# techshoww/RoMa

Measured on AMD Instinct MI355X. Metric: image-pairs/sec at 560->864, higher is better.
Workload: dtype fp16; 1 GPU; roma_outdoor 560->864 full coarse-to-fine symmetric match (BASELINE configs[1]; configs[2] = --pairs 8 --gpus 8); launch=eager launches, coarse_res=560, upsample_res=864, parallelism=single GPU

## Files before the change

include/roma_hip.h:

```cpp
#ifndef ROMA_HIP_H
#define ROMA_HIP_H

#include <stdint.h>

#ifdef __cplusplus
extern "C" {
#endif

#define ROMA_ABI_VERSION 5

enum { ROMA_F32 = 0, ROMA_F16 = 1, ROMA_BF16 = 2 };
enum { ROMA_NCHW = 0, ROMA_NHWC = 1 };
enum { ROMA_LC_AUTO = 0, ROMA_LC_TILE8X4 = 1, ROMA_LC_TILE8X8 = 2, ROMA_LC_ROWS8 = 3 };
enum { ROMA_E_ARG = -1, ROMA_E_DTYPE = -2, ROMA_E_SHAPE = -3, ROMA_E_ALIGN = -4, ROMA_E_UNSUPPORTED = -5 };

int roma_abi_version(void);
const char* roma_last_error(void);

int roma_local_corr(const void* f0, const void* f1, const float* flow, void* out,
                    int B, int C, int H, int W, int r, int dtype,
                    int layout, int f0_pitch, int f1_pitch, int out_layout, int out_pitch, int f1_batch_shift, int variant,
                    void* stream);

int roma_warp_bilinear(const void* src, const float* flow, void* dst,
                       int B, int C, int Hs, int Ws, int H, int W, int dtype,
                       int layout, int src_pitch, int dst_layout, int dst_pitch, int src_batch_shift, void* stream);

int roma_disp_emb(const float* flow, const float* weight, const float* bias, void* dst,
                  int B, int E, int H, int W, float gain, int dtype, int dst_layout, int dst_pitch, void* stream);

int roma_interp_bilinear(const float* x, float* y, int N, int Hi, int Wi, int Ho, int Wo, void* stream);

int roma_flow_update(float* flow, float* cert, const float* cert_in, const float* delta,
                     int B, int H, int W, float sx, float sy, void* stream);

int roma_cls_to_flow_refine(const void* logits, float* flow_out, float* cert_out,
                            int B, int C, int HW, long stride_b, long stride_c, long stride_p,
                            int dtype, void* stream);

int roma_cos_kernel(const void* x, const void* y, float* K, int B, int N, int M, int D, int dtype, int x_pitch, int y_pitch,
                    int y_batch_shift, float T, float eps, float diag_add, void* stream);

int roma_chol_diag_block(float* A, int lda, long strideA, float* W, int ldw, long strideW, int nb, int B, int* info,
                         int info_base, void* stream);

int roma_chol_step(float* A, int lda, long strideA, int n, int ncols, int j, int nb, const float* W, int ldw, long strideW, float* R,
                   int ldr, long strideR, float* Wn, int ldwn, long strideWn, int* info, int info_base, int B, void* stream);

int roma_chol_subst_step(int dir, const float* W, int ldw, long strideW, const float* R, long strideRb, long strideRs, int ldr, float* T,
                         long strideTb, long strideTs, int ldt, int t_in_panel, float* X, int ldx, long strideX, int n, int m, int nb,
                         int s, int B, void* stream);

int roma_attention_fwd(const void* q, const void* k, const void* v, void* o, int B, int H, int Nq, int Nk, int head_dim, long q_sb,
                       long q_sn, long q_sh, long k_sb, long k_sn, long k_sh, long v_sb, long v_sn, long v_sh, long o_sb, long o_sn,
                       long o_sh, float scale, int dtype, void* stream);

int roma_match_finalize(const float* flow, const float* cert, const float* cert16, float* warp, float* certainty,
                        int P, int H, int W, int H16, int W16, int symmetric, void* stream);

int roma_kde_density(const float* x, float* density, int N, int down, float std, int half_mode, void* stream);

int roma_race_keys(const float* p, const long* counter, float* keys, long N, float thresh, unsigned seed, unsigned stage,
                   void* stream);

int roma_nn_argmin(const float* q, const float* r, int* idx, int NQ, int NR, void* stream);

int roma_resample_u8(const void* in, void* out, int H, int W, int C, int out_size, int axis, const int* bounds,
                     const int* coef, int ksize, void* stream);
int roma_normalize_u8(const void* in, float* out, int H, int W, const float* mean3, const float* std3, void* stream);

int roma_bias_relu_nchw(void* x, const void* bias, int B, int C, int HW, int dtype, void* stream);

int roma_bias_relu_pool2_nchw(void* x, const void* bias, void* pooled, int B, int C, int H, int W, int dtype, void* stream);

int roma_bias_relu_nhwc(void* x, const void* bias, long npix, int C, int dtype, void* stream);
int roma_bias_relu_pool2_nhwc(void* x, const void* bias, void* pooled, int B, int C, int H, int W, int dtype, void* stream);

int roma_dwconv5x5_bn_relu(const void* x, const float* w, const float* scale, const float* shift, void* y,
                           int B, int C, int H, int W, int dtype, int x_pitch, int y_pitch, void* stream);

int roma_refiner_block(const void* x, const void* w25, const float* scale, const float* shift, const void* wt,
                       const float* bias, void* y, int B, int C, int H, int W, int kpad, int dtype, int x_pitch, int y_pitch,
                       void* stream);

int roma_refiner_wide_pack(const void* wt, void* wp, int D);
int roma_refiner_wide_taps(const void* w25, void* w25p, int D);
int roma_refiner_block_wide(const void* x, const void* w25p, const float* scale, const float* shift, const void* wp,
                            const float* bias, void* y, int B, int H, int W, int D, int x_pitch, int y_pitch, int dtype,
                            void* stream);

int roma_pointwise_mfma(const void* x, const void* wt, const float* bias, void* y, long M, int C, int kpad, int dtype,
                        int x_pitch, int y_pitch, void* stream);

int roma_refiner_head(const void* x, const float* wo, const float* bo, float* flow, const float* cert_in, float* cert_out,
                      float* delta_out, int B, int H, int W, int C, int pitch, int dtype, float sx, float sy, void* stream);

int roma_pointwise_small(const void* x, const float* wt, const float* bias, void* y, long M, int C, int dtype,
                         int x_pitch, int y_pitch, void* stream);

int roma_add_layernorm(void* x, int x_dtype, long x_stride, const void* y, int y_dtype, long y_stride, const float* ls,
                       const float* gamma, const float* beta, void* out, int out_dtype, long out_stride, long rows, int C,
                       float eps, void* stream);

int roma_tiny_corr_posembed(const float* f0, const float* f1, float* out, int B, int C,
                            int H0, int W0, int H1, int W1, int exact, void* stream);

int roma_jpeg_info(const void* data, long nbytes, int* info);
int roma_jpeg_entropy_decode(const void* data, long nbytes, int16_t* coef, uint16_t* qt);
int roma_jpeg_reconstruct(const int16_t* coef, const uint16_t* qt, void* planes, void* rgb, const int* info, void* stream);

long roma_ransac_workspace(int kind, int P, int N, int iters, long* offsets);
int roma_ransac_hypotheses(int kind, const double* xa, const double* xb, int P, int N, int iters, float threshold, unsigned seed,
                           int p0, void* ws, long ws_bytes, void* stream);
int roma_ransac_select(int kind, const double* xa, const double* xb, int P, int N, int iters, float threshold, int lo_iters,
                       const void* ws, long ws_bytes, double* model, unsigned char* mask, void* stream);

#ifdef __cplusplus
}
#endif
#endif
```

roma_amd/_lib.py:

```python
from __future__ import annotations

import ctypes
import os
from ctypes import c_char_p, c_float, c_int, c_long, c_void_p

_HERE = os.path.dirname(os.path.abspath(__file__))
LIB_PATH = os.path.join(_HERE, "csrc", "libroma_hip.so")

ROMA_F32, ROMA_F16, ROMA_BF16 = 0, 1, 2
ROMA_NCHW, ROMA_NHWC = 0, 1
LC_VARIANTS = {"auto": 0, "tile8x4": 1, "tile8x8": 2, "rows8": 3}
ABI_VERSION = 5
ROMA_E_ARG, ROMA_E_DTYPE, ROMA_E_SHAPE, ROMA_E_ALIGN, ROMA_E_UNSUPPORTED = -1, -2, -3, -4, -5

SIGNATURES = {
    "roma_abi_version": [],
    "roma_last_error": [],
    "roma_local_corr": [c_void_p, c_void_p, c_void_p, c_void_p, c_int, c_int, c_int, c_int, c_int, c_int,
                        c_int, c_int, c_int, c_int, c_int, c_int, c_int, c_void_p],
    "roma_warp_bilinear": [c_void_p, c_void_p, c_void_p, c_int, c_int, c_int, c_int, c_int, c_int, c_int,
                           c_int, c_int, c_int, c_int, c_int, c_void_p],
    "roma_disp_emb": [c_void_p, c_void_p, c_void_p, c_void_p, c_int, c_int, c_int, c_int, c_float, c_int, c_int, c_int, c_void_p],
    "roma_interp_bilinear": [c_void_p, c_void_p, c_int, c_int, c_int, c_int, c_int, c_void_p],
    "roma_flow_update": [c_void_p, c_void_p, c_void_p, c_void_p, c_int, c_int, c_int, c_float, c_float, c_void_p],
    "roma_cls_to_flow_refine": [c_void_p, c_void_p, c_void_p, c_int, c_int, c_int, c_long, c_long, c_long, c_int, c_void_p],
    "roma_cos_kernel": [c_void_p, c_void_p, c_void_p, c_int, c_int, c_int, c_int, c_int, c_int, c_int, c_int, c_float, c_float,
                        c_float, c_void_p],
    "roma_add_layernorm": [c_void_p, c_int, c_long, c_void_p, c_int, c_long, c_void_p, c_void_p, c_void_p, c_void_p, c_int, c_long,
                           c_long, c_int, c_float, c_void_p],
    "roma_attention_fwd": [c_void_p, c_void_p, c_void_p, c_void_p, c_int, c_int, c_int, c_int, c_int] + [c_long] * 12 + [c_float, c_int, c_void_p],
    "roma_chol_diag_block": [c_void_p, c_int, c_long, c_void_p, c_int, c_long, c_int, c_int, c_void_p, c_int, c_void_p],
    "roma_chol_step": [c_void_p, c_int, c_long, c_int, c_int, c_int, c_int, c_void_p, c_int, c_long, c_void_p, c_int, c_long,
                       c_void_p, c_int, c_long, c_void_p, c_int, c_int, c_void_p],
    "roma_chol_subst_step": [c_int, c_void_p, c_int, c_long, c_void_p, c_long, c_long, c_int, c_void_p, c_long, c_long, c_int, c_int,
                             c_void_p, c_int, c_long, c_int, c_int, c_int, c_int, c_int, c_void_p],
    "roma_match_finalize": [c_void_p, c_void_p, c_void_p, c_void_p, c_void_p, c_int, c_int, c_int, c_int, c_int, c_int, c_void_p],
    "roma_kde_density": [c_void_p, c_void_p, c_int, c_int, c_float, c_int, c_void_p],
    "roma_nn_argmin": [c_void_p, c_void_p, c_void_p, c_int, c_int, c_void_p],
    "roma_race_keys": [c_void_p, c_void_p, c_void_p, c_long, c_float, ctypes.c_uint, ctypes.c_uint, c_void_p],
    "roma_dwconv5x5_bn_relu": [c_void_p, c_void_p, c_void_p, c_void_p, c_void_p, c_int, c_int, c_int, c_int, c_int, c_int, c_int, c_void_p],
    "roma_resample_u8": [c_void_p, c_void_p, c_int, c_int, c_int, c_int, c_int, c_void_p, c_void_p, c_int, c_void_p],
    "roma_normalize_u8": [c_void_p, c_void_p, c_int, c_int, c_void_p, c_void_p, c_void_p],
    "roma_bias_relu_nchw": [c_void_p, c_void_p, c_int, c_int, c_int, c_int, c_void_p],
    "roma_bias_relu_pool2_nchw": [c_void_p, c_void_p, c_void_p, c_int, c_int, c_int, c_int, c_int, c_void_p],
    "roma_bias_relu_nhwc": [c_void_p, c_void_p, c_long, c_int, c_int, c_void_p],
    "roma_bias_relu_pool2_nhwc": [c_void_p, c_void_p, c_void_p, c_int, c_int, c_int, c_int, c_int, c_void_p],
    "roma_pointwise_mfma": [c_void_p, c_void_p, c_void_p, c_void_p, c_long, c_int, c_int, c_int, c_int, c_int, c_void_p],
    "roma_refiner_block": [c_void_p, c_void_p, c_void_p, c_void_p, c_void_p, c_void_p, c_void_p, c_int, c_int, c_int, c_int, c_int, c_int,
                           c_int, c_int, c_void_p],
    "roma_refiner_wide_pack": [c_void_p, c_void_p, c_int],
    "roma_refiner_wide_taps": [c_void_p, c_void_p, c_int],
    "roma_jpeg_info": [c_void_p, c_long, c_void_p],
    "roma_jpeg_entropy_decode": [c_void_p, c_long, c_void_p, c_void_p],
    "roma_jpeg_reconstruct": [c_void_p, c_void_p, c_void_p, c_void_p, c_void_p, c_void_p],
    "roma_refiner_block_wide": [c_void_p, c_void_p, c_void_p, c_void_p, c_void_p, c_void_p, c_void_p, c_int, c_int, c_int, c_int, c_int, c_int,
                                c_int, c_void_p],
    "roma_refiner_head": [c_void_p, c_void_p, c_void_p, c_void_p, c_void_p, c_void_p, c_void_p, c_int, c_int, c_int, c_int, c_int, c_int,
                          c_float, c_float, c_void_p],
    "roma_pointwise_small": [c_void_p, c_void_p, c_void_p, c_void_p, c_long, c_int, c_int, c_int, c_int, c_void_p],
    "roma_tiny_corr_posembed": [c_void_p, c_void_p, c_void_p, c_int, c_int, c_int, c_int, c_int, c_int, c_int, c_void_p],
    "roma_ransac_workspace": [c_int, c_int, c_int, c_int, c_void_p],
    "roma_ransac_hypotheses": [c_int, c_void_p, c_void_p, c_int, c_int, c_int, c_float, ctypes.c_uint, c_int, c_void_p, c_long, c_void_p],
    "roma_ransac_select": [c_int, c_void_p, c_void_p, c_int, c_int, c_int, c_float, c_int, c_void_p, c_long, c_void_p, c_void_p,
                           c_void_p],
}
_RESTYPES = {"roma_last_error": c_char_p, "roma_ransac_workspace": c_long}

_lib = None


class RomaHipError(RuntimeError):
    pass


def load() -> ctypes.CDLL:
    global _lib
    if _lib is not None:
        return _lib
    if not os.path.exists(LIB_PATH):
        raise RomaHipError(f"{LIB_PATH} is missing: build it with `python -c 'import __graft_entry__ as g; g.build()'` "
                           f"or `make -C roma_amd/csrc`.  roma_amd has no CPU/PyTorch fallback for its kernels.")
    lib = ctypes.CDLL(LIB_PATH)
    for name, argtypes in SIGNATURES.items():
        fn = getattr(lib, name)
        fn.argtypes = argtypes
        fn.restype = _RESTYPES.get(name, c_int)
    if lib.roma_abi_version() != ABI_VERSION:
        raise RomaHipError(f"libroma_hip.so ABI {lib.roma_abi_version()} != binding ABI {ABI_VERSION}")
    _lib = lib
    return lib


def check(rc: int, what: str):
    if rc == 0:
        return
    msg = load().roma_last_error().decode(errors="replace")
    if rc < 0:
        raise ValueError(f"{what}: {msg} (code {rc})")
    raise RomaHipError(f"{what}: HIP error {rc}: {msg}")
```

roma_amd/matcher.py:

```python
from __future__ import annotations

import math
import os
from typing import Dict, Optional
from warnings import warn

import numpy as np
import torch
import torch.nn as nn
import torch.nn.functional as F

from . import ops
from .transformer import Block, TransformerDecoder

IMAGENET_MEAN = (0.485, 0.456, 0.406)
IMAGENET_STD = (0.229, 0.224, 0.225)


def _round_up(n, m):
    return (n + m - 1) // m * m


def pixel_grid(b, h, w, device):
    ys = torch.linspace(-1 + 1 / h, 1 - 1 / h, h, device=device)
    xs = torch.linspace(-1 + 1 / w, 1 - 1 / w, w, device=device)
    return torch.stack((xs[None, :].expand(h, w), ys[:, None].expand(h, w)), dim=0)[None].expand(b, 2, h, w).contiguous()


def _params_version(module):
    return tuple((p.data_ptr(), 0 if p.is_inference() else p._version) for p in list(module.parameters()) + list(module.buffers()))


def _zero_pad(t, *shape):
    out = torch.zeros(shape, dtype=t.dtype, device=t.device)
    out[tuple(slice(0, s) for s in t.shape)] = t
    return out


class ConvRefiner(nn.Module):

    def __init__(self, in_dim, hidden_dim, out_dim, hidden_blocks, displacement_emb_dim, local_corr_radius=None,
                 amp_dtype=torch.float16):
        super().__init__()
        assert in_dim == hidden_dim, "depthwise refiner blocks keep the channel count (all shipped models)"

        def block(i, o):
            return nn.Sequential(nn.Conv2d(i, o, 5, 1, 2, groups=i), nn.BatchNorm2d(o), nn.ReLU(inplace=True), nn.Conv2d(o, o, 1, 1, 0))

        self.block1 = block(in_dim, hidden_dim)
        self.hidden_blocks = nn.Sequential(*[block(hidden_dim, hidden_dim) for _ in range(hidden_blocks)])
        self.out_conv = nn.Conv2d(hidden_dim, out_dim, 1, 1, 0)
        self.disp_emb = nn.Conv2d(2, displacement_emb_dim, 1, 1, 0)
        self.has_displacement_emb = True
        self.local_corr_radius = local_corr_radius
        self.in_dim, self.out_dim = in_dim, out_dim
        self.amp_dtype = amp_dtype
        self._prep = None

    def prepare(self, dtype):
        key = (dtype, _params_version(self))
        if self._prep is not None and self._prep[0] == key:
            return self._prep[1]
        D = self.in_dim
        Dp = _round_up(D, 64) if D > 160 else _round_up(D, 8)
        dev = self.out_conv.weight.device
        fuse_max = int(os.environ.get("ROMA_FUSED_BLOCK", "32"))
        fused = Dp <= min(fuse_max, 160) and dtype in (torch.float16, torch.bfloat16)
        mid = (not fused) and 32 < Dp <= 160 and dtype in (torch.float16, torch.bfloat16) and os.environ.get("ROMA_PW_MFMA", "1") != "0"
        wide = Dp == 576 and dtype == torch.float16 and os.environ.get("ROMA_WIDE_BLOCK", "1") != "0"
        blocks = []
        for blk in [self.block1] + list(self.hidden_blocks):
            dw, bn, _, pw = blk
            s = bn.weight.float() / torch.sqrt(bn.running_var.float() + bn.eps)
            w25 = torch.zeros(25, Dp, device=dev)
            w25[:, :D] = dw.weight.float().reshape(D, 25).t()
            scale = torch.zeros(Dp, device=dev)
            shift = torch.zeros(Dp, device=dev)
            scale[:D] = s
            b_dw = dw.bias.float() if dw.bias is not None else torch.zeros(D, device=dev)
            shift[:D] = (b_dw - bn.running_mean.float()) * s + bn.bias.float()
            wt = torch.zeros(Dp, Dp, device=dev)
            wt[:D, :D] = pw.weight.float().reshape(D, D).t()
            b = torch.zeros(Dp, device=dev)
            b[:D] = pw.bias.float()
            if wide:
                blocks.append((w25.contiguous(), scale, shift, wt.to(dtype).contiguous(), b.to(dtype),
                               ops.refiner_wide_taps(w25, dtype), ops.refiner_wide_pack(wt.t().contiguous().to(dtype)), b.contiguous()))
            elif fused:
                kp = 32 if Dp <= 32 else 160
                blocks.append((_zero_pad(w25, 25, kp).to(dtype), _zero_pad(scale, kp), _zero_pad(shift, kp),
                               _zero_pad(wt.t(), kp, kp).to(dtype), _zero_pad(b, kp)))
            elif mid:
                blocks.append((w25.contiguous(), scale, shift, _zero_pad(wt.t(), 160, 160).to(dtype), _zero_pad(b, 160)))
            elif Dp <= 32:
                blocks.append((w25.contiguous(), scale, shift, wt.contiguous(), b.contiguous()))
            else:
                blocks.append((w25.contiguous(), scale, shift, wt.to(dtype).contiguous(), b.to(dtype)))
        wo = torch.zeros(Dp, self.out_dim, device=dev)
        wo[:D] = self.out_conv.weight.float().reshape(self.out_dim, D).t()
        prep = dict(D=D, Dp=Dp, fused=fused, mid=mid, wide=wide, blocks=blocks, wo=wo.contiguous(), bo=self.out_conv.bias.float(),
                    we=self.disp_emb.weight.float().reshape(-1, 2).contiguous(), be=self.disp_emb.bias.float())
        self._prep = (key, prep)
        return prep

    def new_buffer(self, B, h, w, dtype, device):
        return torch.empty((B, h, w, self.prepare(dtype)["Dp"]), dtype=dtype, device=device)

    @torch.no_grad()
    def _body(self, x, y, flow, scale_factor, dtype, buf=None, batch_shift=0):
        P = self.prepare(dtype)
        B, C, h, w = x.shape
        D, Dp = P["D"], P["Dp"]
        E = P["we"].shape[0]
        r = self.local_corr_radius
        K = (2 * r + 1) ** 2 if r else 0
        assert 2 * C + E + K == D, "feature width does not match this refiner"
        x_in_place = buf is not None
        if buf is None:
            buf = torch.empty((B, h, w, Dp), dtype=dtype, device=x.device)
        assert buf.shape == (B, h, w, Dp) and buf.dtype == dtype and buf.is_contiguous()
        d = buf.permute(0, 3, 1, 2)
        if x_in_place:
            assert x.data_ptr() == buf.data_ptr() and x.stride(1) == 1, "x must already be channels [0, C) of buf"
        else:
            d[:, :C].copy_(x)
        if Dp > D:
            buf[..., D:].zero_()
        yy = y.to(dtype)
        ops.warp_bilinear(yy, flow, out=d[:, C:2 * C], batch_shift=batch_shift)
        ops.disp_emb(flow, P["we"], P["be"], 40 / 32 * scale_factor, out=d[:, 2 * C:2 * C + E])
        if r:
            ops.local_correlation(d[:, :C], yy, r, flow=flow, out=d[:, 2 * C + E:D], batch_shift=batch_shift)
        M = B * h * w
        cur = buf
        if P["wide"] and B * ((h + 7) // 8) * ((w + 15) // 16) >= 2 * 256:
            nxt = torch.empty_like(buf)
            for blk in P["blocks"]:
                ops.refiner_block_wide(cur, blk[5], blk[1], blk[2], blk[6], blk[7], out=nxt)
                cur, nxt = nxt, cur
            return cur, P
        if P["fused"]:
            nxt = torch.empty_like(buf)
            for (w25, scale, shift, wt, b) in P["blocks"]:
                ops.refiner_block(cur, w25, scale, shift, wt, b, Dp, out=nxt)
                cur, nxt = nxt, cur
            return cur, P
        for blk in P["blocks"]:
            w25, scale, shift, wt, b = blk[:5]
            t = ops.dwconv5x5_bn_relu(cur.permute(0, 3, 1, 2), w25, scale, shift)
            rows = t.permute(0, 2, 3, 1).reshape(M, Dp)
            if P["mid"]:
                cur = ops.pointwise_mfma(rows, wt, b, Dp)
            else:
                cur = ops.pointwise_small(rows, wt, b) if Dp <= 32 else torch.addmm(b, rows, wt)
            cur = cur.view(B, h, w, Dp)
        return cur, P

    @torch.no_grad()
    def forward(self, x, y, flow, scale_factor=1, logits=None, dtype=None):
        flow = flow.float().contiguous()
        cur, P = self._body(x, y, flow, scale_factor, dtype or self.amp_dtype)
        B, h, w, Dp = cur.shape
        out = torch.addmm(P["bo"], cur.reshape(B * h * w, Dp).float(), P["wo"])
        out = out.view(B, h, w, self.out_dim).permute(0, 3, 1, 2).contiguous()
        return out[:, :-1], out[:, -1:]

    @torch.no_grad()
    def forward_update(self, x, y, flow, certainty, scale_factor, sx, sy, dtype=None, buf=None, batch_shift=0):
        cur, P = self._body(x, y, flow, scale_factor, dtype or self.amp_dtype, buf=buf, batch_shift=batch_shift)
        return ops.refiner_head(cur, P["wo"], P["bo"], flow, certainty, sx, sy)


class CosKernel(nn.Module):
    def __init__(self, T=0.2, learn_temperature=False):
        super().__init__()
        self.T = T

    def __call__(self, x, y, eps=1e-6):
        return ops.cos_kernel(x, y, T=self.T, eps=eps)


class GP(nn.Module):

    def __init__(self, gp_dim=512, T=0.2, sigma_noise=0.1, kernel=None, **_):
        super().__init__()
        self.K = CosKernel(T=T)
        self.sigma_noise = sigma_noise
        self.pos_conv = nn.Conv2d(2, gp_dim, 1, 1)
        self.dim = gp_dim
        self._basis = {}

    def basis(self, b, h, w, device):
        key = (h, w, device, _params_version(self.pos_conv))
        f = self._basis.get(key)
        if f is None:
            g = pixel_grid(1, h, w, device)
            f = torch.cos(8 * math.pi * F.conv2d(g, self.pos_conv.weight.float(), self.pos_conv.bias.float()))
            f = f.flatten(2).transpose(1, 2).contiguous()
            self._basis = {key: f}
        return f.expand(b, -1, -1)

    @torch.no_grad()
    def forward(self, x, y, **kwargs):
        b, c, h1, w1 = x.shape
        _, _, h2, w2 = y.shape
        xs = x.float().flatten(2).transpose(1, 2).contiguous()
        ys = y.float().flatten(2).transpose(1, 2).contiguous()
        K_yy = ops.cos_kernel(ys, ys, T=self.K.T, diag_add=self.sigma_noise)
        K_xy = ops.cos_kernel(xs, ys, T=self.K.T)
        mu = self.posterior_product(K_xy, ops.spd_solve(K_yy, self.basis(1, h2, w2, x.device)))
        return mu.transpose(1, 2).reshape(b, self.dim, h1, w1)

    def posterior_rows(self, xs, ys, h2, w2, fp64=False, batch_shift=0, out=None, check="now"):
        B, n = xs.shape[0], xs.shape[1]
        s = batch_shift % B
        basis = self.basis(1, h2, w2, xs.device)
        if fp64:
            a = xs.double()
            c = (a.roll(-s, 0) if s else a) if ys is None else ys.double()

            def cosk(u, v):
                g = torch.einsum("bnd,bmd->bnm", u, v) / (u.norm(dim=-1)[..., None] * v.norm(dim=-1)[:, None] + 1e-6)
                return ((g - 1.0) / self.K.T).exp()

            Kyy = cosk(c, c) + self.sigma_noise * torch.eye(c.shape[1], device=c.device, dtype=torch.float64)
            Z = torch.cholesky_solve(basis.double().expand(B, -1, -1), torch.linalg.cholesky(Kyy))
            mu = (cosk(a, c) @ Z).float()
            if out is not None:
                out.copy_(mu)
                return out
            return mu
        if ys is None:
            K_self = ops.cos_kernel(xs, xs, T=self.K.T, diag_add=self.sigma_noise)
            K_xy = ops.cos_kernel(xs, xs, T=self.K.T, batch_shift=s)
            Z = ops.spd_solve(K_self, basis, check=check)
            if s:
                assert 2 * s == B, "only the half swap of forward_symmetric"
                Z = torch.cat((Z[s:], Z[:s]), dim=0)
        else:
            K_yy = ops.cos_kernel(ys, ys, T=self.K.T, diag_add=self.sigma_noise)
            K_xy = ops.cos_kernel(xs, ys, T=self.K.T)
            Z = ops.spd_solve(K_yy, basis, check=check)
        return self.posterior_product(K_xy, Z, out)

    @staticmethod
    def posterior_product(K_xy, Z, out=None):
        mu = torch.bmm(K_xy.double(), Z.double())
        if out is None:
            return mu.float()
        out.copy_(mu)
        return out


class Decoder(nn.Module):
    def __init__(self, embedding_decoder, gps, proj, conv_refiner, detach=True, scales=("16", "8", "4", "2", "1"),
                 amp_dtype=torch.float16, **_):
        super().__init__()
        self.embedding_decoder, self.gps, self.proj, self.conv_refiner = embedding_decoder, gps, proj, conv_refiner
        self.scales = list(scales)
        self.refine_init = 4
        self.amp_dtype = amp_dtype
        self.gp_precision = "fp32"
        self.record = None
        self.flow_override = None
        self._proj = None

    def _embedding_decoder_for(self, dtype):
        if dtype == torch.float32:
            return self.embedding_decoder
        key = (dtype, _params_version(self.embedding_decoder))
        hit = self.__dict__.get("_embed_cast")
        if hit is None or hit[0] != key:
            import copy
            with torch.inference_mode(False), torch.no_grad():
                cp = copy.deepcopy(self.embedding_decoder).eval()
                for m in cp.modules():
                    if isinstance(m, nn.Linear):
                        m.to(dtype)
                hit = (key, cp)
            self.__dict__["_embed_cast"] = hit
        return hit[1]

    def get_placeholder_flow(self, b, h, w, device):
        return pixel_grid(b, h, w, device)

    def folded_proj(self, dtype):
        key = (dtype, _params_version(self.proj))
        if self._proj is not None and self._proj[0] == key:
            return self._proj[1]
        out = {}
        for s, seq in self.proj.items():
            conv, bn = seq[0], seq[1]
            g = bn.weight.float() / torch.sqrt(bn.running_var.float() + bn.eps)
            wt = (conv.weight.float().reshape(conv.out_channels, -1) * g[:, None]).t().contiguous().to(dtype)
            b = ((conv.bias.float() - bn.running_mean.float()) * g + bn.bias.float()).to(dtype)
            out[s] = (wt, b)
            if wt.shape[1] < 16:
# ... 348 lines not shown
```

roma_amd/ops.py:

```python
from __future__ import annotations

import math
from typing import Optional

import torch

from . import _lib
from ._lib import ROMA_BF16, ROMA_F16, ROMA_F32, ROMA_NCHW, ROMA_NHWC, check

_DT = {torch.float32: ROMA_F32, torch.float16: ROMA_F16, torch.bfloat16: ROMA_BF16}


class KernelTimer:

    def __init__(self):
        self.enabled = False
        self.bracket_overhead_s = 0.0
        self.records = []

    def start(self):
        self.records.clear()
        torch.cuda.synchronize()
        pairs = []
        for _ in range(32):
# ... 366 lines not shown
    p = p.reshape(-1).float().contiguous()
    if counter is not None:
        counter = counter.reshape(-1).long().contiguous()
        assert counter.numel() == p.numel()
    keys = torch.empty_like(p)
    check(_lib.load().roma_race_keys(_p(p), _p(counter), _p(keys), p.numel(), float(thresh), int(seed) & 0xFFFFFFFF,
                                     int(stage) & 0xFFFFFFFF, _stream()), "roma_race_keys")
    return keys


def nn_argmin(q, r):
    _need_gpu(q, r)
    if q.dim() != 2 or q.shape[1] != 2 or r.dim() != 2 or r.shape[1] != 2:
        raise ValueError("nn_argmin expects (N,2) point sets")
    q, r = q.float().contiguous(), r.float().contiguous()
    idx = torch.empty((q.shape[0],), dtype=torch.int32, device=q.device)
    check(_lib.load().roma_nn_argmin(_p(q), _p(r), _p(idx), q.shape[0], r.shape[0], _stream()), "roma_nn_argmin")
    return idx.long()


def dwconv5x5_bn_relu(x, w25, scale, shift, out=None):
    _need_gpu(x, w25, scale, shift, out)
    B, C, H, W = x.shape
    lx, px, xx = feat_layout(x)
    if lx != ROMA_NHWC:
        raise ValueError("dwconv5x5_bn_relu needs channels-last input")
    if out is None:
        out = nhwc_empty(B, C, H, W, x.dtype, x.device, pitch=px)
    lo, po, o = feat_layout(out)
    if lo != ROMA_NHWC or o is not out:
        raise ValueError("dwconv5x5_bn_relu needs channels-last output")
    check(_lib.load().roma_dwconv5x5_bn_relu(_p(xx), _p(w25), _p(scale), _p(shift), _p(out), B, C, H, W, _dt(xx), px, po, _stream()),
          "roma_dwconv5x5_bn_relu")
    return out


def resample_u8(img, out_size, axis, bounds, coef, ksize):
    _need_gpu(img, bounds, coef)
    H, W, C = img.shape
    assert img.dtype == torch.uint8 and img.is_contiguous() and bounds.dtype == torch.int32 and coef.dtype == torch.int32
    assert bounds.shape == (out_size, 2) and coef.shape == (out_size, ksize) and bounds.is_contiguous() and coef.is_contiguous()
    out = torch.empty((H, out_size, C) if axis else (out_size, W, C), dtype=torch.uint8, device=img.device)
    check(_lib.load().roma_resample_u8(_p(img), _p(out), H, W, C, out_size, axis, _p(bounds), _p(coef), ksize, _stream()), "roma_resample_u8")
    return out


def normalize_u8(img, mean, std):
    import ctypes
    _need_gpu(img)
    H, W, C = img.shape
    assert C == 3 and img.dtype == torch.uint8 and img.is_contiguous()
    out = torch.empty((3, H, W), dtype=torch.float32, device=img.device)
    m = (ctypes.c_float * 3)(*mean)
    s = (ctypes.c_float * 3)(*std)
    check(_lib.load().roma_normalize_u8(_p(img), _p(out), H, W, ctypes.cast(m, ctypes.c_void_p), ctypes.cast(s, ctypes.c_void_p), _stream()),
          "roma_normalize_u8")
    return out


def _is_nhwc(x):
    return x.dim() == 4 and x.shape[1] > 1 and x.stride(1) == 1 and x.is_contiguous(memory_format=torch.channels_last)


def bias_relu_(x, bias):
    _need_gpu(x, bias)
    B, C, H, W = x.shape
    assert bias.dtype == x.dtype and bias.numel() == C and bias.is_contiguous()
    if _is_nhwc(x):
        check(_lib.load().roma_bias_relu_nhwc(_p(x), _p(bias), B * H * W, C, _dt(x), _stream()), "roma_bias_relu_nhwc")
        return x
    assert x.is_contiguous()
    step = max(1, 65535 // C)
    for b0 in range(0, B, step):
        xb = x[b0:b0 + step]
        check(_lib.load().roma_bias_relu_nchw(_p(xb), _p(bias), xb.shape[0], C, H * W, _dt(x), _stream()), "roma_bias_relu_nchw")
    return x


def bias_relu_pool2_(x, bias):
    _need_gpu(x, bias)
    B, C, H, W = x.shape
    assert bias.dtype == x.dtype and bias.numel() == C and bias.is_contiguous() and H % 2 == 0 and W % 2 == 0
    if _is_nhwc(x):
        out = torch.empty((B, H // 2, W // 2, C), dtype=x.dtype, device=x.device).permute(0, 3, 1, 2)
        check(_lib.load().roma_bias_relu_pool2_nhwc(_p(x), _p(bias), _p(out), B, C, H, W, _dt(x), _stream()), "roma_bias_relu_pool2_nhwc")
        return out
    assert x.is_contiguous()
    out = torch.empty((B, C, H // 2, W // 2), dtype=x.dtype, device=x.device)
    step = max(1, 65535 // C)
    for b0 in range(0, B, step):
        xb = x[b0:b0 + step]
        check(_lib.load().roma_bias_relu_pool2_nchw(_p(xb), _p(bias), _p(out[b0:b0 + step]), xb.shape[0], C, H, W, _dt(x), _stream()),
              "roma_bias_relu_pool2_nchw")
    return out


def pointwise_mfma(rows, wt, bias, C, out=None):
    _need_gpu(rows, wt, bias, out)
    M, pitch = rows.shape
    kpad = wt.shape[0]
    assert rows.is_contiguous() and wt.is_contiguous() and wt.dtype == rows.dtype and bias.numel() == kpad and bias.dtype == torch.float32
    if out is None:
        out = torch.empty_like(rows)
    assert out.shape == rows.shape and out.is_contiguous()
    check(_lib.load().roma_pointwise_mfma(_p(rows), _p(wt), _p(bias), _p(out), M, C, kpad, _dt(rows), pitch, pitch, _stream()),
          "roma_pointwise_mfma")
    return out


def refiner_wide_pack(wt_out_in):
    w = wt_out_in.detach().to("cpu").contiguous()
    assert w.dim() == 2 and w.shape[0] == w.shape[1] and w.element_size() == 2
    out = torch.empty_like(w)
    check(_lib.load().roma_refiner_wide_pack(w.data_ptr(), out.data_ptr(), w.shape[0]), "roma_refiner_wide_pack")
    return out.to(wt_out_in.device)


def refiner_wide_taps(w25, dtype=torch.float16):
    D = w25.shape[1]
    w = w25.detach().to("cpu").to(dtype).contiguous()
    assert w.shape == (25, D) and w.element_size() == 2
    out = torch.empty((D // 32, 5, 4, 2, 6, 4, 2), dtype=dtype)
    check(_lib.load().roma_refiner_wide_taps(w.data_ptr(), out.data_ptr(), D), "roma_refiner_wide_taps")
    return out.to(w25.device)


def refiner_block_wide(x_nhwc, w25p, scale, shift, wp, bias, out=None):
    _need_gpu(x_nhwc, w25p, scale, shift, wp, bias, out)
    B, H, W, D = x_nhwc.shape
    assert x_nhwc.is_contiguous() and w25p.shape == (D // 32, 5, 4, 2, 6, 4, 2) and w25p.dtype == x_nhwc.dtype and w25p.is_contiguous()
    assert all(t.dtype == torch.float32 and t.numel() == D and t.is_contiguous() for t in (scale, shift, bias))
    if out is None:
        out = torch.empty_like(x_nhwc)
    assert out.shape == x_nhwc.shape and out.is_contiguous() and out.data_ptr() != x_nhwc.data_ptr()
    check(_lib.load().roma_refiner_block_wide(_p(x_nhwc), _p(w25p), _p(scale), _p(shift), _p(wp), _p(bias), _p(out), B, H, W, D, D, D,
                                              _dt(x_nhwc), _stream()), "roma_refiner_block_wide")
    return out


def refiner_block(x_nhwc, w25, scale, shift, wt, bias, C, out=None):
    _need_gpu(x_nhwc, w25, scale, shift, wt, bias, out)
    B, h, w, pitch = x_nhwc.shape
    kpad = wt.shape[0]
    assert x_nhwc.is_contiguous() and wt.is_contiguous() and w25.is_contiguous() and wt.dtype == x_nhwc.dtype == w25.dtype
    assert w25.shape == (25, kpad) and wt.shape == (kpad, kpad) and scale.numel() == shift.numel() == bias.numel() == kpad
    if out is None:
        out = torch.empty_like(x_nhwc)
    assert out.is_contiguous() and out.shape == x_nhwc.shape and out.data_ptr() != x_nhwc.data_ptr()
    check(_lib.load().roma_refiner_block(_p(x_nhwc), _p(w25), _p(scale), _p(shift), _p(wt), _p(bias), _p(out), B, C, h, w, kpad,
                                         _dt(x_nhwc), pitch, pitch, _stream()), "roma_refiner_block")
    return out


def refiner_head(x_nhwc, wo, bo, flow, certainty, sx, sy, want_delta=False):
    _need_gpu(x_nhwc, wo, bo, flow, certainty)
    B, h, w, pitch = x_nhwc.shape
    C = wo.shape[0]
    assert x_nhwc.is_contiguous() and flow.is_contiguous() and flow.dtype == torch.float32 and wo.is_contiguous()
    cert_in = None if certainty is None else certainty.float().contiguous()
    cert = torch.empty((B, 1, h, w), dtype=torch.float32, device=flow.device)
    delta = torch.empty((B, 3, h, w), dtype=torch.float32, device=flow.device) if want_delta else None
    check(_lib.load().roma_refiner_head(_p(x_nhwc), _p(wo), _p(bo), _p(flow), _p(cert_in), _p(cert), _p(delta), B, h, w, C, pitch,
                                        _dt(x_nhwc), float(sx), float(sy), _stream()), "roma_refiner_head")
    return (flow, cert, delta) if want_delta else (flow, cert)


def pointwise_small(x_rows, wt, bias, out=None):
    _need_gpu(x_rows, wt, bias, out)
    M, C = x_rows.shape
    assert x_rows.stride(1) == 1
    if out is None:
        out = torch.empty((M, C), dtype=x_rows.dtype, device=x_rows.device)
    check(_lib.load().roma_pointwise_small(_p(x_rows), _p(wt), _p(bias), _p(out), M, C, _dt(x_rows), x_rows.stride(0), out.stride(0),
                                           _stream()), "roma_pointwise_small")
    return out


def attention(qkv, n_valid=None, out=None):
    _need_gpu(qkv, out)
    B, N, three, H, d = qkv.shape
    assert three == 3 and qkv.is_contiguous()
    if out is None:
        out = torch.empty((B, N, H * d), dtype=qkv.dtype, device=qkv.device)
    assert out.is_contiguous() and out.shape == (B, N, H * d) and out.dtype == qkv.dtype
    es = qkv.element_size()
    sb, sn, sh = qkv.stride(0), qkv.stride(1), qkv.stride(3)
    base = qkv.data_ptr()
    step = qkv.stride(2) * es
    check(_lib.load().roma_attention_fwd(base, base + step, base + 2 * step, out.data_ptr(), B, H, N, N if n_valid is None else int(n_valid), d,
                                         sb, sn, sh, sb, sn, sh, sb, sn, sh, out.stride(0), out.stride(1), d, float(d) ** -0.5, _dt(qkv),
                                         _stream()), "roma_attention_fwd")
    return out


def add_layernorm(x, y, ln_weight, ln_bias, eps, out_dtype, ls=None):
    _need_gpu(x, y, ln_weight, ln_bias, ls)
    C = x.shape[-1]
    assert x.is_contiguous() and (y is None or (y.is_contiguous() and y.shape == x.shape))
    rows = x.numel() // C
    out = torch.empty(x.shape, dtype=out_dtype, device=x.device)
    for t in (ln_weight, ln_bias, ls):
        assert t is None or (t.dtype == torch.float32 and t.is_contiguous() and t.numel() == C)
    check(_lib.load().roma_add_layernorm(_p(x), _dt(x), C, _p(y), _dt(y) if y is not None else 0, C, _p(ls), _p(ln_weight), _p(ln_bias),
                                         _p(out), _DT[out_dtype], C, rows, C, float(eps), _stream()), "roma_add_layernorm")
    return out


def tiny_corr_posembed(f0, f1, exact=False):
    _need_gpu(f0, f1)
    B, C, H0, W0 = f0.shape
    _, _, H1, W1 = f1.shape
    a = f0.float().permute(0, 2, 3, 1).contiguous()
    b = f1.float().permute(0, 2, 3, 1).contiguous()
    out = torch.empty((B, 2, H0, W0), dtype=torch.float32, device=f0.device)
    TIMER.wrap("tiny_corr", 2.0 * B * H0 * W0 * H1 * W1 * C, f"C{C}_{H0}x{W0}",
               lambda: check(_lib.load().roma_tiny_corr_posembed(_p(a), _p(b), _p(out), B, C, H0, W0, H1, W1, 1 if exact else 0, _stream()),
                             "roma_tiny_corr_posembed"))
    return out
```

Before: 56.88 image-pairs/s.

## Fuse depthwise 5x5 conv, BN-ReLU and MFMA pointwise for mid-width refiner blocks

```diff
diff --git a/include/roma_hip.h b/include/roma_hip.h
--- a/include/roma_hip.h
+++ b/include/roma_hip.h
@@ -83,6 +83,9 @@
                        const float* bias, void* y, int B, int C, int H, int W, int kpad, int dtype, int x_pitch, int y_pitch,
                        void* stream);
 
+int roma_refiner_mid(const void* x, const float* w25, const float* scale, const float* shift, const void* wt,
+                     const float* bias, void* y, int B, int C, int H, int W, int dtype, int x_pitch, int y_pitch, void* stream);
+
 int roma_refiner_wide_pack(const void* wt, void* wp, int D);
 int roma_refiner_wide_taps(const void* w25, void* w25p, int D);
 int roma_refiner_block_wide(const void* x, const void* w25p, const float* scale, const float* shift, const void* wp,
diff --git a/roma_amd/_lib.py b/roma_amd/_lib.py
--- a/roma_amd/_lib.py
+++ b/roma_amd/_lib.py
@@ -48,6 +48,8 @@
     "roma_pointwise_mfma": [c_void_p, c_void_p, c_void_p, c_void_p, c_long, c_int, c_int, c_int, c_int, c_int, c_void_p],
     "roma_refiner_block": [c_void_p, c_void_p, c_void_p, c_void_p, c_void_p, c_void_p, c_void_p, c_int, c_int, c_int, c_int, c_int, c_int,
                            c_int, c_int, c_void_p],
+    "roma_refiner_mid": [c_void_p, c_void_p, c_void_p, c_void_p, c_void_p, c_void_p, c_void_p, c_int, c_int, c_int, c_int, c_int, c_int, c_int,
+                         c_void_p],
     "roma_refiner_wide_pack": [c_void_p, c_void_p, c_int],
     "roma_refiner_wide_taps": [c_void_p, c_void_p, c_int],
     "roma_jpeg_info": [c_void_p, c_long, c_void_p],
diff --git a/roma_amd/csrc/refiner_mid.hip b/roma_amd/csrc/refiner_mid.hip
--- /dev/null
+++ b/roma_amd/csrc/refiner_mid.hip
@@ -0,0 +1,288 @@
+#include <algorithm>
+#include <cstdlib>
+#include "common.h"
+
+namespace roma {
+namespace {
+
+typedef _Float16 h8v __attribute__((ext_vector_type(8)));
+
+constexpr int RM_NT = 512;
+constexpr int RM_KPAD = 160, RM_KS = 5;
+constexpr int RM_RS = RM_KPAD / 8 + 1;
+constexpr int RM_OS = RM_KPAD + 8;
+constexpr int RM_XT = 16;
+constexpr int RM_RMAX = 16;
+
+struct RMParams {
+  const half_t* x;
+  half_t* y;
+  const float* w25;
+  const half_t* wt;
+  const float* scale;
+  const float* shift;
+  const float* bias;
+  int B, H, W, C, x_pitch, y_pitch;
+  int R;
+  int tiles_x, tiles_y, ntile;
+};
+
+inline int rm_rows(int C, int xs, int ys) { return std::min(RM_RMAX, RM_NT / (C / 8) / (RM_XT / xs) * ys); }
+inline int rm_trows(int R) { return (R + 1) & ~1; }
+inline size_t rm_smem(int C, int R) {
+  return (size_t)RM_KPAD * RM_RS * 16 + (size_t)rm_trows(R) * RM_XT * RM_OS * 2 + (size_t)25 * C * 4 + (size_t)3 * RM_KPAD * 4;
+}
+
+template <int RM_XS, int RM_YS, int RM_PD>
+__global__ __launch_bounds__(RM_NT, 1) void refiner_mid_kernel(RMParams p) {
+  constexpr int RM_NC = RM_XS + 4, NSX = RM_XT / RM_XS;
+  extern __shared__ __attribute__((aligned(16))) unsigned char smem[];
+  u32x4* s_pw = reinterpret_cast<u32x4*>(smem);
+  half_t* s_t = reinterpret_cast<half_t*>(s_pw + RM_KPAD * RM_RS);
+  float* s_w = reinterpret_cast<float*>(s_t + ((p.R + 1) & ~1) * RM_XT * RM_OS);
+  float* s_cs = s_w + 25 * p.C;
+  const int tid = threadIdx.x, lane = tid & 63;
+  const int wv = __builtin_amdgcn_readfirstlane(tid >> 6);
+  const int m = lane & 15, kq = lane >> 4;
+  const int C = p.C, H = p.H, W = p.W, R = p.R;
+  const int PK = C >> 3;
+
+  for (int i = tid; i < RM_KPAD * (RM_KPAD / 8); i += RM_NT) {
+    const int n = i / (RM_KPAD / 8), k = i - n * (RM_KPAD / 8);
+    s_pw[n * RM_RS + k] = reinterpret_cast<const u32x4*>(p.wt)[i];
+  }
+  for (int i = tid; i < 25 * C / 4; i += RM_NT) reinterpret_cast<float4_t*>(s_w)[i] = reinterpret_cast<const float4_t*>(p.w25)[i];
+  for (int i = tid; i < RM_KPAD; i += RM_NT) {
+    s_cs[i] = i < C ? p.scale[i] : 0.f;
+    s_cs[RM_KPAD + i] = i < C ? p.shift[i] : 0.f;
+    s_cs[2 * RM_KPAD + i] = p.bias[i];
+  }
+  {
+    const int npad = RM_KPAD / 8 - PK;
+    for (int i = tid; i < R * RM_XT * npad; i += RM_NT) {
+      const int px = i / npad, k = PK + (i - px * npad);
+      *reinterpret_cast<u32x4*>(s_t + px * RM_OS + k * 8) = u32x4{0, 0, 0, 0};
+    }
+  }
+
+  int row, sx, k;
+  {
+    const int s = tid / PK;
+    k = tid - s * PK;
+    sx = s % NSX;
+    row = s / NSX * RM_YS;
+  }
+  const bool act = row < R;
+  if (!act) { row = 0; sx = 0; k = 0; }
+  const int c0 = k * 8;
+  const int tpix = row * RM_XT + sx * RM_XS;
+
+  const int ntile = p.ntile, tiles_per_img = p.tiles_x * p.tiles_y;
+  const bool xcd_order = (gridDim.x & 7) == 0 && ntile >= 64;
+  const int nx = xcd_order ? (int)(gridDim.x >> 3) : (int)gridDim.x;
+  const int band = xcd_order ? (ntile + 7) >> 3 : ntile;
+  const int t_beg = xcd_order ? (int)(blockIdx.x & 7) * band + (int)(blockIdx.x >> 3) : (int)blockIdx.x;
+  const int t_end = xcd_order ? min(((int)(blockIdx.x & 7) + 1) * band, ntile) : ntile;
+  auto tile_origin = [&](int tile, int& b, int& ty0, int& tx0) {
+    b = tile / tiles_per_img;
+    const int tt = tile - b * tiles_per_img, tyi = tt / p.tiles_x;
+    ty0 = tyi * R;
+    tx0 = (tt - tyi * p.tiles_x) * RM_XT;
+  };
+  const char* xc = reinterpret_cast<const char*>(p.x);
+  auto load_row_clamped = [&](u32x4 (&dst)[RM_NC], int b, int yi, int xi0) {
+    const unsigned ro = (unsigned)((b * H + min(max(yi, 0), H - 1)) * W);
+#pragma unroll
+    for (int cx = 0; cx < RM_NC; ++cx)
+      dst[cx] = *reinterpret_cast<const u32x4*>(xc + ((ro + (unsigned)min(max(xi0 + cx, 0), W - 1)) * (unsigned)p.x_pitch + (unsigned)c0) * 2u);
+  };
+
+  constexpr int NR = RM_YS + 4, PD = RM_PD;
+  u32x4 q[PD][RM_NC];
+  {
+    int b, ty0, tx0;
+    tile_origin(min(t_beg, ntile - 1), b, ty0, tx0);
+#pragma unroll
+    for (int j = 0; j < PD; ++j) load_row_clamped(q[j], b, ty0 + row + j - 2, tx0 + sx * RM_XS - 2);
+  }
+  __syncthreads();
+
+  const u32x4* t_rd = reinterpret_cast<const u32x4*>(s_t + (2 * wv * RM_XT + m) * RM_OS) + kq;
+  const u32x4* pw_rd = s_pw + m * RM_RS + kq;
+  const float* bias_rd = s_cs + 2 * RM_KPAD + m;
+  half_t* o_wr = s_t + (2 * wv * RM_XT + 4 * kq) * RM_OS + m;
+  const int NTL = (C + 15) >> 4;
+
+  for (int tile = t_beg; tile < t_end; tile += nx) {
+    int b, ty0, tx0;
+    tile_origin(tile, b, ty0, tx0);
+    const int ys = ty0 + row, xs = tx0 + sx * RM_XS;
+    float acc[RM_YS][RM_XS][8];
+#pragma unroll
+    for (int oy = 0; oy < RM_YS; ++oy)
+#pragma unroll
+      for (int o = 0; o < RM_XS; ++o)
+#pragma unroll
+        for (int e = 0; e < 8; ++e) acc[oy][o][e] = 0.f;
+    auto fma_row = [&](const u32x4 (&src)[RM_NC], int dy, float (&ac)[RM_XS][8]) {
+#pragma unroll
+      for (int hf = 0; hf < 2; ++hf) {
+        const float* wr = s_w + dy * 5 * C + c0 + 4 * hf;
+        float4_t w5[5];
+#pragma unroll
+        for (int dx = 0; dx < 5; ++dx) w5[dx] = *reinterpret_cast<const float4_t*>(wr + dx * C);
+#pragma unroll
+        for (int cx = 0; cx < RM_NC; ++cx) {
+          float f[4];
+#pragma unroll
+          for (int i = 0; i < 2; ++i) {
+            const uint32_t u = src[cx][2 * hf + i];
+            const half2_t h = __builtin_bit_cast(half2_t, u);
+            f[2 * i] = (float)h[0];
+            f[2 * i + 1] = (float)h[1];
+          }
+#pragma unroll
+          for (int dx = 0; dx < 5; ++dx) {
+            const int o = cx - dx;
+            if (o >= 0 && o < RM_XS) {
+#pragma unroll
+              for (int e = 0; e < 4; ++e) ac[o][4 * hf + e] = __builtin_fmaf(w5[dx][e], f[e], ac[o][4 * hf + e]);
+            }
+          }
+        }
+      }
+    };
+    auto mask_row = [&](u32x4 (&v)[RM_NC], int iy) {
+      const int yi = ys + iy - 2;
+      const bool oky = yi >= 0 && yi < H;
+#pragma unroll
+      for (int cx = 0; cx < RM_NC; ++cx) {
+        const int xi = xs - 2 + cx;
+        if (!(oky && xi >= 0 && xi < W)) v[cx] = u32x4{0, 0, 0, 0};
+      }
+    };
+    const bool interior = ty0 >= 2 && ty0 + R + 2 <= H && tx0 >= 2 && tx0 + RM_XT + 2 <= W;
+    int b2, ty2, tx2;
+    tile_origin(min(tile + nx, t_end - 1), b2, ty2, tx2);
+#pragma unroll 1
+    for (int iy = 0; iy < NR; ++iy) {
+      u32x4 cur[RM_NC];
+#pragma unroll
+      for (int cx = 0; cx < RM_NC; ++cx) cur[cx] = q[0][cx];
+#pragma unroll
+      for (int j = 0; j + 1 < PD; ++j)
+#pragma unroll
+        for (int cx = 0; cx < RM_NC; ++cx) q[j][cx] = q[j + 1][cx];
+      if (!interior) mask_row(cur, iy);
+      const bool mine = iy + PD < NR;
+      load_row_clamped(q[PD - 1], mine ? b : b2, (mine ? ty0 + iy + PD : ty2 + iy + PD - NR) + row - 2, (mine ? tx0 : tx2) + sx * RM_XS - 2);
+      __builtin_amdgcn_sched_barrier(0);
+#pragma unroll
+      for (int oy = 0; oy < RM_YS; ++oy) {
+        const int dy = iy - oy;
+        if (dy >= 0 && dy <= 4) fma_row(cur, dy, acc[oy]);
+      }
+    }
+    if (act) {
+      float sc[8], sh[8];
+#pragma unroll
+      for (int e = 0; e < 8; e += 4) {
+        *reinterpret_cast<float4_t*>(&sc[e]) = *reinterpret_cast<const float4_t*>(s_cs + c0 + e);
+        *reinterpret_cast<float4_t*>(&sh[e]) = *reinterpret_cast<const float4_t*>(s_cs + RM_KPAD + c0 + e);
+      }
+#pragma unroll
+      for (int oy = 0; oy < RM_YS; ++oy)
+#pragma unroll
+        for (int o = 0; o < RM_XS; ++o) {
+          float v[8];
+#pragma unroll
+          for (int e = 0; e < 8; ++e) v[e] = fmaxf(__builtin_fmaf(acc[oy][o][e], sc[e], sh[e]), 0.f);
+          *reinterpret_cast<u32x4*>(s_t + (tpix + oy * RM_XT + o) * RM_OS + c0) = pack16<half_t>(v);
+        }
+    }
+    __syncthreads();
+
+    if (2 * wv < R) {
+      u32x4 a[2][RM_KS];
+#pragma unroll
+      for (int i = 0; i < 2; ++i)
+#pragma unroll
+        for (int ks = 0; ks < RM_KS; ++ks) a[i][ks] = t_rd[i * (RM_XT * RM_OS / 8) + 4 * ks];
+      float4_t pr[2][RM_KPAD / 16];
+#pragma unroll
+      for (int nt = 0; nt < RM_KPAD / 16; ++nt) {
+        pr[0][nt] = pr[1][nt] = float4_t{0.f, 0.f, 0.f, 0.f};
+        if (nt < NTL) {
+#pragma unroll
+          for (int ks = 0; ks < RM_KS; ++ks) {
+            const h8v bfr = __builtin_bit_cast(h8v, pw_rd[nt * 16 * RM_RS + 4 * ks]);
+            pr[0][nt] = __builtin_amdgcn_mfma_f32_16x16x32_f16(__builtin_bit_cast(h8v, a[0][ks]), bfr, pr[0][nt], 0, 0, 0);
+            pr[1][nt] = __builtin_amdgcn_mfma_f32_16x16x32_f16(__builtin_bit_cast(h8v, a[1][ks]), bfr, pr[1][nt], 0, 0, 0);
+          }
+        }
+      }
+#pragma unroll
+      for (int nt = 0; nt < RM_KPAD / 16; ++nt) {
+        if (nt < NTL) {
+          const float bv = bias_rd[nt * 16];
+          if (nt * 16 + m < C)
+#pragma unroll
+          for (int i = 0; i < 2; ++i)
+#pragma unroll
+            for (int r4 = 0; r4 < 4; ++r4) o_wr[(i * RM_XT + r4) * RM_OS + nt * 16] = from_f32<half_t>(pr[i][nt][r4] + bv);
+        }
+      }
+    }
+    __syncthreads();
+    u32x4 ov[RM_YS][RM_XS];
+#pragma unroll
+    for (int oy = 0; oy < RM_YS; ++oy)
+#pragma unroll
+      for (int o = 0; o < RM_XS; ++o) ov[oy][o] = *reinterpret_cast<const u32x4*>(s_t + (tpix + oy * RM_XT + o) * RM_OS + c0);
+    __syncthreads();
+    if (act) {
+#pragma unroll
+      for (int oy = 0; oy < RM_YS; ++oy) {
+        if (ys + oy >= H) break;
+        half_t* yrow = p.y + (((size_t)b * H + ys + oy) * W) * p.y_pitch + c0;
+#pragma unroll
+        for (int o = 0; o < RM_XS; ++o)
+          if (xs + o < W) *reinterpret_cast<u32x4*>(yrow + (size_t)(xs + o) * p.y_pitch) = ov[oy][o];
+      }
+    }
+  }
+}
+
+}
+}
+
+using namespace roma;
+
+extern "C" int roma_refiner_mid(const void* x, const float* w25, const float* scale, const float* shift, const void* wt,
+                                const float* bias, void* y, int B, int C, int H, int W, int dtype, int x_pitch, int y_pitch,
+                                void* stream) {
+  ROMA_REQUIRE(x && w25 && scale && shift && wt && bias && y, ROMA_E_ARG, "roma_refiner_mid: null pointer");
+  ROMA_REQUIRE(x != y, ROMA_E_ARG, "roma_refiner_mid: x and y must not alias");
+  ROMA_REQUIRE(B > 0 && C > 0 && H > 0 && W > 0 && x_pitch >= C && y_pitch >= C, ROMA_E_SHAPE, "roma_refiner_mid: bad shape");
+  ROMA_REQUIRE(dtype == ROMA_F16, ROMA_E_DTYPE, "roma_refiner_mid: fp16 only (bf16 / fp32 use the separate kernels)");
+  ROMA_REQUIRE(C > 32 && C <= RM_KPAD && C % 8 == 0, ROMA_E_UNSUPPORTED, "roma_refiner_mid: C=%d (32 < C <= 160, a multiple of 8)", C);
+  ROMA_REQUIRE(x_pitch % 8 == 0 && y_pitch % 8 == 0 && aligned16(x) && aligned16(y) && aligned16(w25) && aligned16(wt), ROMA_E_ALIGN,
+               "roma_refiner_mid: pitches must be multiples of 8 and bases 16-byte aligned");
+  constexpr int XS = 4, YS = 2, PDEPTH = 2;
+  RMParams p{static_cast<const half_t*>(x), static_cast<half_t*>(y), w25, static_cast<const half_t*>(wt), scale, shift, bias,
+             B, H, W, C, x_pitch, y_pitch, rm_rows(C, XS, YS), 0, 0, 0};
+  p.tiles_x = (W + RM_XT - 1) / RM_XT;
+  p.tiles_y = (H + p.R - 1) / p.R;
+  const long ntile = (long)B * p.tiles_x * p.tiles_y;
+  ROMA_REQUIRE(ntile < (1L << 30) && (size_t)B * H * W * x_pitch * 2 < (1ull << 32), ROMA_E_SHAPE,
+               "roma_refiner_mid: %ld tiles, x of %zu bytes in one launch (< 2^30 tiles, < 4 GB)", ntile, (size_t)B * H * W * x_pitch * 2);
+  p.ntile = (int)ntile;
+  const int smem = (int)rm_smem(C, p.R);
+  static std::atomic<uint64_t> attr_done{0};
+  if (int rc = ensure_dyn_smem(reinterpret_cast<const void*>(refiner_mid_kernel<XS, YS, PDEPTH>), 160 * 1024, attr_done, "roma_refiner_mid")) return rc;
+  const int cus = num_cus();
+  const int per = cus >= 8 ? (cus & ~7) : cus;
+  const int grid = ntile < per ? (int)ntile : per;
+  hipLaunchKernelGGL((refiner_mid_kernel<XS, YS, PDEPTH>), dim3(grid), dim3(RM_NT), smem, static_cast<hipStream_t>(stream), p);
+  ROMA_CHECK_LAUNCH();
+}
diff --git a/roma_amd/matcher.py b/roma_amd/matcher.py
--- a/roma_amd/matcher.py
+++ b/roma_amd/matcher.py
@@ -25,6 +25,13 @@
     ys = torch.linspace(-1 + 1 / h, 1 - 1 / h, h, device=device)
     xs = torch.linspace(-1 + 1 / w, 1 - 1 / w, w, device=device)
     return torch.stack((xs[None, :].expand(h, w), ys[:, None].expand(h, w)), dim=0)[None].expand(b, 2, h, w).contiguous()
+
+
+def _cdiv(a, b):
+    return -(-a // b)
+
+
+MID_BLOCK_MIN_TILES = 180
 
 
 def _params_version(module):
@@ -64,8 +71,7 @@
         D = self.in_dim
         Dp = _round_up(D, 64) if D > 160 else _round_up(D, 8)
         dev = self.out_conv.weight.device
-        fuse_max = int(os.environ.get("ROMA_FUSED_BLOCK", "32"))
-        fused = Dp <= min(fuse_max, 160) and dtype in (torch.float16, torch.bfloat16)
+        fused = Dp <= 32 and dtype in (torch.float16, torch.bfloat16)
         mid = (not fused) and 32 < Dp <= 160 and dtype in (torch.float16, torch.bfloat16) and os.environ.get("ROMA_PW_MFMA", "1") != "0"
         wide = Dp == 576 and dtype == torch.float16 and os.environ.get("ROMA_WIDE_BLOCK", "1") != "0"
         blocks = []
@@ -143,6 +149,13 @@
             nxt = torch.empty_like(buf)
             for (w25, scale, shift, wt, b) in P["blocks"]:
                 ops.refiner_block(cur, w25, scale, shift, wt, b, Dp, out=nxt)
+                cur, nxt = nxt, cur
+            return cur, P
+        if P["mid"] and dtype == torch.float16 and os.environ.get("ROMA_MID_BLOCK", "1") != "0" \
+                and B * _cdiv(h, min(16, 512 // (Dp // 8) // 4 * 2)) * _cdiv(w, 16) >= MID_BLOCK_MIN_TILES:
+            nxt = torch.empty_like(buf)
+            for (w25, scale, shift, wt, b) in P["blocks"]:
+                ops.refiner_block_mid(cur, w25, scale, shift, wt, b, Dp, out=nxt)
                 cur, nxt = nxt, cur
             return cur, P
         for blk in P["blocks"]:
diff --git a/roma_amd/ops.py b/roma_amd/ops.py
--- a/roma_amd/ops.py
+++ b/roma_amd/ops.py
@@ -542,6 +542,20 @@
     return out
 
 
+def refiner_block_mid(x_nhwc, w25, scale, shift, wt, bias, C, out=None):
+    _need_gpu(x_nhwc, w25, scale, shift, wt, bias, out)
+    B, h, w, pitch = x_nhwc.shape
+    assert x_nhwc.is_contiguous() and wt.is_contiguous() and w25.is_contiguous() and wt.dtype == x_nhwc.dtype
+    assert w25.shape == (25, C) and w25.dtype == torch.float32 and wt.shape == (160, 160) and bias.numel() == 160
+    assert all(t.dtype == torch.float32 and t.is_contiguous() for t in (scale, shift, bias)) and scale.numel() == shift.numel() == C
+    if out is None:
+        out = torch.empty_like(x_nhwc)
+    assert out.is_contiguous() and out.shape == x_nhwc.shape and out.data_ptr() != x_nhwc.data_ptr()
+    check(_lib.load().roma_refiner_mid(_p(x_nhwc), _p(w25), _p(scale), _p(shift), _p(wt), _p(bias), _p(out), B, C, h, w,
+                                       _dt(x_nhwc), pitch, pitch, _stream()), "roma_refiner_mid")
+    return out
+
+
 def refiner_head(x_nhwc, wo, bo, flow, certainty, sx, sy, want_delta=False):
     _need_gpu(x_nhwc, wo, bo, flow, certainty)
     B, h, w, pitch = x_nhwc.shape
```

Result: faster. 57.71 image-pairs/s, median of 6 (+1.4%).
